# llGuy/madrona_renderer

Measured on AMD Instinct MI355X. Metric: rendered views/sec (whole node), N worlds x 64x64 RGB+depth, higher is better.
Workload: dtype f32

## Files before the change

madrona_renderer_amd/csrc/raster.hip:

```cpp
#include <hip/hip_runtime.h>
#include <algorithm>
#include <cstdlib>

#include "raster.hpp"
#include "raster_dev.hpp"

namespace mrx {
namespace {

constexpr int kWavesPerBlock = 4;
constexpr int kChunk = 64;
constexpr int kHot = 16;
constexpr int kBandRows = 16;
constexpr int kBlocksPerBand = 16;

struct WaveLds {
    float hot[kChunk][kHot];
    float cold[kChunk][kCold];
};

struct TileCtx {
    uint32_t view, tileX0, tileY0;
    uint32_t triBegin, numTris;
    int lx, ly;
};

__device__ __forceinline__ bool tileSetup(const RasterParams &p, uint32_t item, int lane,
                                          TileCtx &t, ViewConst &vc)
{
    const uint32_t tilesPerView = p.tilesFast * p.tilesSlow;
    if (item >= p.numViews * tilesPerView)
        return false;
    t.view = item / tilesPerView;
    const uint32_t tile = item % tilesPerView;
    t.tileX0 = (tile % p.tilesFast) * 64u;
    t.tileY0 = (tile / p.tilesFast) * 64u;
    const float4 q = *reinterpret_cast<const float4 *>(p.camRot + 4 * t.view);
    quatToMat(q.x, q.y, q.z, q.w, vc.Rc);
#pragma unroll
    for (int r = 0; r < 3; ++r) {
        vc.c[r] = p.camPos[3 * t.view + r];
        vc.lv[r] = dot3(vc.Rc[0][r], vc.Rc[1][r], vc.Rc[2][r],
                        p.toLight[0], p.toLight[1], p.toLight[2]);
    }
#pragma unroll
    for (int r = 0; r < 3; ++r) {
#pragma unroll
        for (int cc = 0; cc < 3; ++cc)
            vc.Rc[r][cc] = __uint_as_float(
                __builtin_amdgcn_readfirstlane(__float_as_uint(vc.Rc[r][cc])));
        vc.c[r] = __uint_as_float(__builtin_amdgcn_readfirstlane(__float_as_uint(vc.c[r])));
        vc.lv[r] = __uint_as_float(__builtin_amdgcn_readfirstlane(__float_as_uint(vc.lv[r])));
    }
    t.triBegin = t.view * p.viewTriStride;
    t.numTris = p.viewTriCount[t.view];
    t.lx = lane & 7;
    t.ly = lane >> 3;
    return true;
}

__device__ __forceinline__ uint64_t setupChunk(const RasterParams &p, const ViewConst &vc,
                                               const TileCtx &t, uint32_t chunk, int lane,
                                               WaveLds &L)
{
    bool valid = false;
    const uint32_t k = chunk + lane;
    if (k < t.numTris) {
        const WorldTri wt = p.viewTris[t.triBegin + k];
        TriPlanes c;
        float *h = L.hot[lane];
        valid = setupTriangle(p, vc, wt, (int32_t)k, c, h + 12, L.cold[lane]);
        h[0] = c.A0; h[1] = c.B0; h[2] = c.C0;
        h[3] = c.A1; h[4] = c.B1; h[5] = c.C1;
        h[6] = c.A2; h[7] = c.B2; h[8] = c.C2;
        h[9] = c.Dx; h[10] = c.Dy; h[11] = c.Dc;
    }
    const uint64_t mask = __ballot(valid);
    waveLdsSync();
    return mask;
}

__device__ __forceinline__ const float *shadeRec(const WaveLds &L, int32_t w) { return &L.hot[w][12]; }

template <bool IDS, typename LDS>
__device__ __forceinline__ void resolvePixel(const RasterParams &p, const LDS &L,
                                             int32_t w, float bestInv, float px, float py,
                                             uint32_t &rgba, int32_t &id)
{
    const float *h = shadeRec(L, w);
    rgba = __float_as_uint(h[0]);
    const int32_t tex = __float_as_int(h[1]);
    if (tex >= 0) {
        const float tt = 1.0f / bestInv;
        rgba = shadeTextured(p, L.cold[w], tex, px, py, tt);
    }
    if (IDS)
        id = __float_as_int(p.idsAreSegmask ? h[2] : h[3]);
}

__device__ __forceinline__ void rasterBandBrute(const WaveLds &L, uint64_t validMask,
                                                const float (&pxf)[8], float py0, float py1,
                                                float invNear,
                                                float (&best)[kBlocksPerBand],
                                                int32_t (&bid)[kBlocksPerBand])
{
    for (uint64_t m = validMask; m != 0; m &= m - 1) {
        const int k = __builtin_ctzll(m);
        const float *h = L.hot[k];
        const float A0 = h[0], B0 = h[1], C0 = h[2];
        const float A1 = h[3], B1 = h[4], C1 = h[5];
        const float A2 = h[6], B2 = h[7], C2 = h[8];
        const float Dx = h[9], Dy = h[10], Dc = h[11];
        float r0[2], r1[2], r2[2], rd[2];
        r0[0] = __builtin_fmaf(B0, py0, C0); r0[1] = __builtin_fmaf(B0, py1, C0);
        r1[0] = __builtin_fmaf(B1, py0, C1); r1[1] = __builtin_fmaf(B1, py1, C1);
        r2[0] = __builtin_fmaf(B2, py0, C2); r2[1] = __builtin_fmaf(B2, py1, C2);
        rd[0] = __builtin_fmaf(Dy, py0, Dc); rd[1] = __builtin_fmaf(Dy, py1, Dc);
#pragma unroll
        for (int b = 0; b < kBlocksPerBand; ++b) {
            const int r = b >> 3, bx = b & 7;
            const float e0 = __builtin_fmaf(A0, pxf[bx], r0[r]);
            const float e1 = __builtin_fmaf(A1, pxf[bx], r1[r]);
            const float e2 = __builtin_fmaf(A2, pxf[bx], r2[r]);
            const float it = __builtin_fmaf(Dx, pxf[bx], rd[r]);
            const bool in = (fminf(fminf(e0, e1), e2) >= 0.0f) &&
                            (it > best[b]) && (it <= invNear);
            best[b] = in ? it : best[b];
            bid[b] = in ? k : bid[b];
        }
    }
}

template <bool IDS, bool MULTI, int OUT = kOutRGBD>
__global__ __launch_bounds__(kWave *kWavesPerBlock)
void rasterBruteKernel(const RasterParams p)
{
    __shared__ WaveLds lds[kWavesPerBlock];
    touchKernelArguments();
    const int wave = threadIdx.x / kWave;
    const int lane = threadIdx.x % kWave;
    TileCtx t;
    ViewConst vc;
    if (!tileSetup(p, blockIdx.x * kWavesPerBlock + wave, lane, t, vc))
        return;
    WaveLds &L = lds[wave];

    float pxf[8];
#pragma unroll
    for (int bx = 0; bx < 8; ++bx)
        pxf[bx] = (float)(t.tileX0 + bx * 8 + t.lx);
    const float invNear = p.invNear;

    uint64_t mask0 = 0;
    if (!MULTI)
        mask0 = setupChunk(p, vc, t, 0, lane, L);

    for (int band = 0; band < 4; ++band) {
        float best[kBlocksPerBand];
        int32_t bid[kBlocksPerBand];
        uint32_t outRgba[kBlocksPerBand];
        int32_t outId[kBlocksPerBand];
#pragma unroll
        for (int b = 0; b < kBlocksPerBand; ++b) {
            best[b] = p.invFar;
            bid[b] = -1;
            outRgba[b] = 0xFF000000u;
            outId[b] = -1;
        }
        const float py0 = (float)(t.tileY0 + band * kBandRows + t.ly);
        const float py1 = (float)(t.tileY0 + band * kBandRows + 8 + t.ly);

        if (!MULTI) {
            rasterBandBrute(L, mask0, pxf, py0, py1, invNear, best, bid);
#pragma unroll
            for (int b = 0; b < kBlocksPerBand; ++b)
                if (bid[b] >= 0)
                    resolvePixel<IDS>(p, L, bid[b], best[b], pxf[b & 7],
                                      (b >> 3) ? py1 : py0, outRgba[b], outId[b]);
        } else {
            for (uint32_t chunk = 0; chunk < t.numTris; chunk += kChunk) {
                const uint64_t mask = setupChunk(p, vc, t, chunk, lane, L);
                rasterBandBrute(L, mask, pxf, py0, py1, invNear, best, bid);
#pragma unroll
                for (int b = 0; b < kBlocksPerBand; ++b) {
                    if (bid[b] >= 0)
                        resolvePixel<IDS>(p, L, bid[b], best[b], pxf[b & 7],
                                          (b >> 3) ? py1 : py0, outRgba[b], outId[b]);
                    bid[b] = -1;
                }
                waveLdsSync();
            }
        }

#pragma unroll
        for (int b = 0; b < kBlocksPerBand; ++b) {
            const int r = b >> 3, bx = b & 7;
            const uint32_t fx = t.tileX0 + bx * 8 + t.lx;
            const uint32_t fy = t.tileY0 + band * kBandRows + r * 8 + t.ly;
            if (fx < p.nfast && fy < p.nslow) {
                const bool hit = best[b] > p.invFar;
                const float dep = hit ? 1.0f / best[b] : 0.0f;
                const size_t o = ((size_t)t.view * p.nslow + fy) * p.nfast + fx;
                if (OUT != kOutDepth)
                    p.rgb[o] = outRgba[b];
                if (OUT != kOutRGB)
                    p.depth[o] = dep;
                if (IDS)
                    p.ids[o] = outId[b];
            }
        }
    }
}

constexpr uint32_t kNearFree = 1u << 16;

template <int S0, int S1>
__device__ __forceinline__ uint32_t classifyStrips(const TriPlanes &c, uint32_t tileX0,
                                                   uint32_t tileY0, float invNear, float invFar,
                                                   bool &nearOk)
{
    const float X0 = (float)tileX0, Y0 = (float)tileY0;
    const float xa0 = c.A0 < 0.0f ? X0 : X0 + 31.0f;
    const float xa1 = c.A1 < 0.0f ? X0 : X0 + 31.0f;
    const float xa2 = c.A2 < 0.0f ? X0 : X0 + 31.0f;
    const float xdh = c.Dx < 0.0f ? X0 : X0 + 31.0f;
    const float xdl = c.Dx < 0.0f ? X0 + 31.0f : X0;
    const float yb0 = c.B0 < 0.0f ? Y0 : Y0 + 7.0f;
    const float yb1 = c.B1 < 0.0f ? Y0 : Y0 + 7.0f;
    const float yb2 = c.B2 < 0.0f ? Y0 : Y0 + 7.0f;
    const float ydh = c.Dy < 0.0f ? Y0 : Y0 + 7.0f;
    const float ydl = c.Dy < 0.0f ? Y0 + 7.0f : Y0;
    uint32_t mask = 0;
    float dmax = -__builtin_inff();
#pragma unroll
    for (int s = S0; s < S1; ++s) {
        const float dy = (float)(8 * s);
        const float r0 = __builtin_fmaf(c.B0, yb0 + dy, c.C0);
        const float r1 = __builtin_fmaf(c.B1, yb1 + dy, c.C1);
        const float r2 = __builtin_fmaf(c.B2, yb2 + dy, c.C2);
        const float rh = __builtin_fmaf(c.Dy, ydh + dy, c.Dc);
        const float rl = __builtin_fmaf(c.Dy, ydl + dy, c.Dc);
        const bool yin = (Y0 + dy + 7.0f >= c.bbY0) && (Y0 + dy <= c.bbY1);
#pragma unroll
        for (int hf = 0; hf < 2; ++hf) {
            const float dx = (float)(32 * hf);
            const float e0 = __builtin_fmaf(c.A0, xa0 + dx, r0);
            const float e1 = __builtin_fmaf(c.A1, xa1 + dx, r1);
            const float e2 = __builtin_fmaf(c.A2, xa2 + dx, r2);
            const float dh = __builtin_fmaf(c.Dx, xdh + dx, rh);
            const float dl = __builtin_fmaf(c.Dx, xdl + dx, rl);
            const bool xin = (X0 + dx + 31.0f >= c.bbX0) && (X0 + dx <= c.bbX1);
            const bool possible = (fminf(fminf(e0, e1), e2) >= 0.0f) &&
                                  (dh > invFar) && (dl <= invNear) && xin && yin;
            mask |= possible ? (1u << (2 * s + hf)) : 0u;
            dmax = fmaxf(dmax, dh);
        }
    }
    nearOk = dmax <= invNear;
    return mask;
}

__device__ __forceinline__ uint32_t classifyRegions(const TriPlanes &c, const TileCtx &t,
                                                    float invNear, float invFar)
{
    bool nearOk;
    uint32_t mask = classifyStrips<0, 8>(c, t.tileX0, t.tileY0, invNear, invFar, nearOk);
    if (nearOk)
        mask |= kNearFree;
    return mask;
}


template <bool NEAR>
__device__ __forceinline__ void pixelTest(const PlanePairs &q, f32x2 r01, f32x2 r2d, float px,
                                          float invNear, int32_t kv, float &best, int32_t &bid)
{
    const f32x2 pp = { px, px };
    const f32x2 e01 = fma2(q.A01, pp, r01);
    const f32x2 e2d = fma2(q.A2D, pp, r2d);
    bool in = (fminf(fminf(e01.x, e01.y), e2d.x) >= 0.0f) & (e2d.y > best);
    if (NEAR)
        in = in & (e2d.y <= invNear);
    best = in ? e2d.y : best;
    bid = in ? kv : bid;
}

template <bool NEAR, int IDSHIFT>
__device__ __forceinline__ void rasterRegion(const float (*planes)[16], uint64_t act, int recBase,
                                             const float (&px)[kRegionBlocks], float py,
                                             float invNear,
                                             float (&best)[kRegionBlocks],
                                             int32_t (&bid)[kRegionBlocks])
{
    const f32x2 yy = { py, py };
    for (; act != 0; act &= act - 1) {
        const int k = recBase + __builtin_ctzll(act);
        const PlanePairs q = loadPlanes(planes, k);
        const f32x2 r01 = fma2(q.B01, yy, q.C01);
        const f32x2 r2d = fma2(q.B2D, yy, q.C2D);
#pragma unroll
        for (int b = 0; b < kRegionBlocks; ++b)
            pixelTest<NEAR>(q, r01, r2d, px[b], invNear, k << IDSHIFT, best[b], bid[b]);
    }
}

template <bool IDS>
__device__ __forceinline__ void outputRegion(const RasterParams &p, const TileCtx &t,
                                             uint32_t fx0, uint32_t fy, float invFar,
                                             const float (&best)[kRegionBlocks],
                                             const uint32_t (&rgba)[kRegionBlocks],
                                             const int32_t (&id)[kRegionBlocks])
{
    float dep[kRegionBlocks];
#pragma unroll
    for (int b = 0; b < kRegionBlocks; ++b)
        dep[b] = best[b] > invFar ? __builtin_amdgcn_rcpf(best[b]) : 0.0f;
    if (fy >= p.nslow || (p.debugSkip & 1u))
        return;
    const size_t o = ((size_t)t.view * p.nslow + fy) * p.nfast + fx0;
    const bool doRgb = storesRgb<kOutByPointer>(p.rgb), doDepth = storesDepth<kOutByPointer>(p.depth);
    if ((p.nfast & 3u) == 0 && fx0 + 3 < p.nfast) {
        if (doRgb)
            streamStore16(p.writeThrough, p.rgb + o, rgba[0], rgba[1], rgba[2], rgba[3]);
        if (doDepth)
            streamStore16(p.writeThrough, p.depth + o, __float_as_uint(dep[0]), __float_as_uint(dep[1]),
                          __float_as_uint(dep[2]), __float_as_uint(dep[3]));
        if (IDS)
            streamStore16(p.writeThrough, p.ids + o, (uint32_t)id[0], (uint32_t)id[1], (uint32_t)id[2], (uint32_t)id[3]);
    } else {
#pragma unroll
        for (int b = 0; b < kRegionBlocks; ++b) {
            if (fx0 + b < p.nfast) {
                if (doRgb)
                    streamStore4(p.writeThrough, p.rgb + o + b, rgba[b]);
                if (doDepth)
                    streamStore4(p.writeThrough, p.depth + o + b, __float_as_uint(dep[b]));
                if (IDS)
                    streamStore4(p.writeThrough, p.ids + o + b, (uint32_t)id[b]);
            }
        }
    }
}

constexpr int kPass = kChunk * kWavesPerBlock;

struct PassRecs {
    float shade[kPass][4];
    float cold[kPass][kCold];
};
struct TileLds {
    float planes[kPass][16];
    PassRecs rec;
};
__device__ __forceinline__ const float *shadeRec(const PassRecs &L, int32_t w) { return L.shade[w]; }

template <bool IDS>
__global__ __launch_bounds__(kWave *kWavesPerBlock, 3)
void rasterChunkedKernel(const RasterParams p)
{
    __shared__ TileLds lds;
    touchKernelArguments();
    const int wave = threadIdx.x / kWave;
    const int lane = threadIdx.x % kWave;
    TileCtx t;
    ViewConst vc;
    if (!tileSetup(p, blockIdx.x, lane, t, vc))
        return;
    const float invNear = p.invNear, invFar = p.invFar;

    float best[4][kRegionBlocks];
    int32_t bid[4][kRegionBlocks];
    uint32_t outRgba[4][kRegionBlocks];
    int32_t outId[4][kRegionBlocks];
#pragma unroll
    for (int g = 0; g < 4; ++g)
#pragma unroll
        for (int b = 0; b < kRegionBlocks; ++b) {
            best[g][b] = invFar;
            bid[g][b] = -1;
            outRgba[g][b] = 0xFF000000u;
            outId[g][b] = -1;
        }

    for (uint32_t pass = 0; pass < t.numTris; pass += kPass) {
        if (pass != 0)
            __syncthreads();
        {
            const int rec = wave * kWave + lane;
            const uint32_t k = pass + (uint32_t)rec;
            TriPlanes c;
            c.A0 = c.B0 = c.C0 = c.A1 = c.B1 = c.C1 = 0.0f;
            c.A2 = c.B2 = c.C2 = c.Dx = c.Dy = c.Dc = 0.0f;
            c.bbX0 = c.bbX1 = c.bbY0 = c.bbY1 = 0.0f;
            uint32_t mask = 0;
            if (pass + (uint32_t)(wave * kWave) < t.numTris) {
                bool valid = false;
                if (k < t.numTris && !(p.debugSkip & 8u)) {
                    const WorldTri wt = p.viewTris[t.triBegin + k];
                    valid = setupTriangle(p, vc, wt, (int32_t)k, c, lds.rec.shade[rec], lds.rec.cold[rec]);
                }
                if (valid && !(p.debugSkip & 4u))
                    mask = classifyRegions(c, t, invNear, invFar);
            }
            float4 *dst = reinterpret_cast<float4 *>(lds.planes[rec]);
            dst[0] = make_float4(c.A0, c.A1, c.A2, c.Dx);
            dst[1] = make_float4(c.B0, c.B1, c.B2, c.Dy);
            dst[2] = make_float4(c.C0, c.C1, c.C2, c.Dc);
            dst[3] = make_float4(__uint_as_float(mask), 0.f, 0.f, 0.f);
        }
        __syncthreads();

        const uint32_t left = t.numTris - pass;
        const int subs = left >= (uint32_t)kPass ? kWavesPerBlock : (int)((left + kWave - 1) / kWave);
#pragma unroll
        for (int g = 0; g < 4; ++g) {
            const int strip = 2 * wave + (g >> 1), hf = g & 1;
            const uint32_t fy = t.tileY0 + strip * 8 + t.ly;
            const float py = (float)fy;
            const uint32_t fx0 = t.tileX0 + hf * 32 + 4 * t.lx;
            float px[kRegionBlocks];
#pragma unroll
            for (int b = 0; b < kRegionBlocks; ++b)
                px[b] = (float)(fx0 + b);
            for (int sub = 0; sub < subs; ++sub) {
                const uint32_t mask = __float_as_uint(lds.planes[sub * kWave + lane][12]);
                const uint64_t act = __ballot((mask >> (2 * strip + hf)) & 1u);
                if (!(p.debugSkip & 2u))
                    rasterRegion<true, 0>(lds.planes, act, sub * kWave, px, py, invNear, best[g], bid[g]);
            }
#pragma unroll
            for (int b = 0; b < kRegionBlocks; ++b) {
                if (bid[g][b] >= 0)
                    resolvePixel<IDS>(p, lds.rec, bid[g][b], best[g][b], px[b], py,
                                      outRgba[g][b], outId[g][b]);
                bid[g][b] = -1;
            }
        }
    }

#pragma unroll
    for (int g = 0; g < 4; ++g) {
        const int strip = 2 * wave + (g >> 1), hf = g & 1;
        const uint32_t fy = t.tileY0 + strip * 8 + t.ly;
        const uint32_t fx0 = t.tileX0 + hf * 32 + 4 * t.lx;
        outputRegion<IDS>(p, t, fx0, fy, invFar, best[g], outRgba[g], outId[g]);
    }
}

constexpr int kGroupTilesMax = 16;
constexpr int kGroupSlotsMax = 256;
constexpr int groupTilesMax(int slots) { return slots <= 128 ? kGroupTilesMax : 8; }

template <int SLOTS>
struct GroupLds {
    static constexpr int kRecs = SLOTS <= kChunk ? kChunk + 16 : SLOTS;
    static constexpr int kBackground = kRecs;
    float planes[kRecs][16];
    uint32_t live[kRecs];
    float shade[kRecs + 1][4];
    float cold[kRecs][kCold];
    uint32_t masks[groupTilesMax(SLOTS) * (SLOTS <= kChunk ? kChunk : SLOTS)];
    uint32_t tileInfo[kGroupTilesMax][4];
    uint32_t nextItem;
    uint8_t itemOrder[kGroupTilesMax * 8];
};
constexpr uint32_t kTileValid = 4u;


template <bool IDS, bool FULL, bool TEX, int OUT, typename LDS>
__device__ __forceinline__ void storeRegion(const RasterParams &p, const LDS &L, bool doRgb, bool doDepth,
                                            uint32_t *rgbTile, float *depthTile, int32_t *idsTile,
                                            uint32_t pixOff, uint32_t fx0, uint32_t fy,
                                            bool anyTex, const float (&px)[kRegionBlocks], float py,
                                            const float (&best)[kRegionBlocks],
                                            const int32_t (&bid)[kRegionBlocks])
{
    uint32_t rgba[kRegionBlocks];
    int32_t id[kRegionBlocks];
    float dep[kRegionBlocks];
    const char *shadeBase = reinterpret_cast<const char *>(&L.shade[0][0]);
#pragma unroll
    for (int b = 0; b < kRegionBlocks; ++b) {
        const float *h = reinterpret_cast<const float *>(shadeBase + bid[b]);
        if (OUT != kOutDepth)
            rgba[b] = __float_as_uint(h[0]);
        if (IDS)
            id[b] = __float_as_int(p.idsAreSegmask ? h[2] : h[3]);
        if (OUT != kOutRGB)
            dep[b] = bid[b] != LDS::kBackground * 16 ? __builtin_amdgcn_rcpf(best[b]) : 0.0f;
    }
    if (TEX && OUT != kOutDepth && anyTex && (OUT != kOutByPointer || doRgb)) {
#pragma unroll
        for (int b = 0; b < kRegionBlocks; ++b) {
            const int32_t rec = bid[b] >> 4;
            const int32_t tex = __float_as_int(L.shade[rec][1]);
            if (tex >= 0)
                rgba[b] = shadeTextured(p, L.cold[rec], tex, px[b], py, 1.0f / best[b]);
        }
    }
    if (p.debugSkip & 1u)
        return;
    if (FULL) {
        if (doRgb)
            streamStore16(p.writeThrough, rgbTile + pixOff, rgba[0], rgba[1], rgba[2], rgba[3]);
        if (doDepth)
            streamStore16(p.writeThrough, depthTile + pixOff, __float_as_uint(dep[0]), __float_as_uint(dep[1]),
                          __float_as_uint(dep[2]), __float_as_uint(dep[3]));
        if (IDS)
            streamStore16(p.writeThrough, idsTile + pixOff, (uint32_t)id[0], (uint32_t)id[1], (uint32_t)id[2], (uint32_t)id[3]);
    } else if (fy < p.nslow) {
#pragma unroll
        for (int b = 0; b < kRegionBlocks; ++b) {
            if (fx0 + b < p.nfast) {
                if (doRgb)
                    streamStore4(p.writeThrough, rgbTile + pixOff + b, rgba[b]);
                if (doDepth)
                    streamStore4(p.writeThrough, depthTile + pixOff + b, __float_as_uint(dep[b]));
                if (IDS)
                    streamStore4(p.writeThrough, idsTile + pixOff + b, (uint32_t)id[b]);
            }
        }
    }
}

template <bool IDS, bool FULL>
__device__ __forceinline__ void storeBackground(const RasterParams &p, bool doRgb, bool doDepth, uint32_t *rgbTile,
                                                float *depthTile, int32_t *idsTile,
                                                uint32_t pixOff, uint32_t fx0, uint32_t fy)
{
    if (p.debugSkip & 1u)
        return;
    const uint32_t bg = 0xFF000000u;
    if (FULL) {
        if (doRgb)
            streamStore16(p.writeThrough, rgbTile + pixOff, bg, bg, bg, bg);
        if (doDepth)
            streamStore16(p.writeThrough, depthTile + pixOff, 0u, 0u, 0u, 0u);
        if (IDS)
            streamStore16(p.writeThrough, idsTile + pixOff, ~0u, ~0u, ~0u, ~0u);
    } else if (fy < p.nslow) {
#pragma unroll
        for (int b = 0; b < kRegionBlocks; ++b) {
            if (fx0 + b < p.nfast) {
                if (doRgb)
                    streamStore4(p.writeThrough, rgbTile + pixOff + b, bg);
                if (doDepth)
                    streamStore4(p.writeThrough, depthTile + pixOff + b, 0u);
                if (IDS)
                    streamStore4(p.writeThrough, idsTile + pixOff + b, ~0u);
            }
        }
    }
}

struct GroupSetupArgs {
    const ObjTri *tris;
    const TriMat *triMats;
    const float *instPos, *instRot, *instScale;
    float sx, ox, sz, oz, s6bPad, ambient, diffuse;
    int32_t transposed;
};

constexpr int groupWaves(bool tex) { return tex ? 4 : 8; }

template <bool IDS, int SLOTS, bool TEX, int XMODE, bool FAST, int OUT>
__device__ __forceinline__ void groupKernelBody(const char *hPose, const char *hGeom, uint32_t hViews, uint32_t hInstances,
                                                uint32_t hPool, uint32_t hShape, uint32_t hGroups, uint32_t hPrefix,
                                                uint32_t hFirst01, uint32_t hFirst23, const RasterParams p)
{
    __shared__ GroupLds<SLOTS> lds;
    constexpr int kBackground = GroupLds<SLOTS>::kBackground;
    const int wave = __builtin_amdgcn_readfirstlane(threadIdx.x / kWave);
    const int lane = threadIdx.x % kWave;
    if (!FAST || wave >= 2)
        touchKernelArguments<(FAST ? 48 : 0) + sizeof(RasterParams)>();
    const uint32_t aNumViews = FAST ? hViews : p.numViews;
    const uint32_t aGrpViews = FAST ? (hShape & 255u) : p.grpViews;
    const uint32_t aXcdSkew = FAST ? ((hShape >> 8) & 15u) : p.xcdSkew;
    const uint32_t aXcdRotate = FAST ? ((hShape >> 12) & 1u) : p.xcdRotate;
    const uint32_t aGrpPerView = FAST ? 1u : p.grpPerView;
    const uint32_t aGrid = FAST ? hGroups : gridDim.x;
    const uint32_t aUniInstances = FAST ? ((hShape >> 13) & 7u) : p.uniInstances;
    const uint32_t aUniCams = FAST ? ((hShape >> 16) & 255u) : p.uniCamsPerWorld;
    const uint32_t dskip = FAST ? 0u : p.debugSkip;
    const PoseLayout lay = poseLayout(hViews, hInstances);
    const float *aCamRot = FAST ? reinterpret_cast<const float *>(hPose + lay.camRot) : p.camRot;
    const float *aCamPos = FAST ? reinterpret_cast<const float *>(hPose + lay.camPos) : p.camPos;
    const int32_t *aInstObj = FAST ? reinterpret_cast<const int32_t *>(hPose + lay.instObj) : p.instObj;
    const uint32_t tilesPerView = FAST ? 1u : p.tilesFast * p.tilesSlow;
    uint32_t firstView, groupViews, firstTile, groupTiles;
    const uint32_t blk = ((XMODE & 1) && SLOTS == 16 && aXcdSkew && (blockIdx.x ^ 1u) < aGrid)
                             ? blockIdx.x ^ 1u : blockIdx.x;
    if ((XMODE & 2) && blockIdx.x == 0 && threadIdx.x == (groupWaves(TEX) - 1) * kWave && p.xccReport)
        *p.xccReport = __builtin_amdgcn_s_getreg((3 << 11) | 20);
    uint32_t bid = blk;
    if (aXcdRotate && (bid | 7u) < aGrid)
        bid = (bid & ~7u) | ((bid + 2u * (bid >> 3)) & 7u);
    if (aGrpPerView == 1) {
        firstView = bid * aGrpViews;
        groupViews = aGrpViews;
        firstTile = 0;
        groupTiles = groupViews * tilesPerView;
    } else {
        firstView = bid / aGrpPerView;
        groupViews = 1;
        firstTile = (bid - firstView * aGrpPerView) * p.grpChunkTiles;
        groupTiles = min(p.grpChunkTiles, tilesPerView - firstTile);
    }
    uint32_t firstStrip = 0, numStrips = groupTiles * 8;
    if (SLOTS == 16 && aXcdSkew) {
        if (blk & 1u) {
            firstStrip = aXcdSkew;
            numStrips -= aXcdSkew;
        } else {
            groupViews += 1;
            groupTiles += 1;
            numStrips += aXcdSkew;
        }
    }
    const int groupRecs = (int)groupViews * SLOTS;
    const int numPairs = (int)groupTiles * SLOTS;
    const float invNear = p.invNear, invFar = p.invFar;
    if (dskip & 16u)
        return;
    unsigned long long *stamps = (!FAST && p.debugStamps && wave < 4)
        ? p.debugStamps + ((size_t)blockIdx.x * 4 + wave) * 8 : nullptr;
#define MRX_STAMP(i)                                                           \
    do {                                                                       \
        if (stamps && lane == 0)                                               \
            stamps[i] = __builtin_amdgcn_s_memrealtime();                      \
    } while (0)
    MRX_STAMP(0);
    for (int i = threadIdx.x; i < numPairs; i += groupWaves(TEX) * kWave)
        lds.masks[i] = 0u;

    if (wave == groupWaves(TEX) - 1 && lane < (int)groupTiles) {
        uint32_t vi = (uint32_t)lane, tile = firstTile;
        if (tilesPerView != 1) {
            vi = groupViews == 1 ? 0u : (uint32_t)lane / tilesPerView;
            tile = firstTile + (uint32_t)lane - vi * tilesPerView;
        }
        const uint32_t ty = tilesPerView != 1 ? tile / p.tilesFast : 0u;
        lds.tileInfo[lane][0] = firstView + vi;
        lds.tileInfo[lane][1] = (tile - ty * p.tilesFast) * 64u;
        lds.tileInfo[lane][2] = ty * 64u;
        lds.tileInfo[lane][3] = (firstView + vi < aNumViews ? kTileValid : 0u) | ((vi * SLOTS) << 8);
    }
    if (wave == groupWaves(TEX) - 1) {
        uint32_t base = 0;
        for (uint32_t c0 = 0; c0 < groupTiles * 8u; c0 += kWave) {
            const uint32_t c = c0 + (uint32_t)lane;
            uint32_t strip = c / groupTiles, tile = c - strip * groupTiles;
            if (tilesPerView != 1) {
                tile = c >> 3;
                strip = c & 7u;
            }
            const uint32_t g = tile * 8u + strip;
            const bool ok = strip < 8u && g >= firstStrip && g < firstStrip + numStrips;
            const uint64_t m = __ballot(ok);
            if (ok)
                lds.itemOrder[base + __builtin_popcountll(m & ((1ull << lane) - 1ull))] = (uint8_t)g;
            base += (uint32_t)__builtin_popcountll(m);
        }
    }
    if (wave * kWave < groupRecs) {
        const int rec = wave * kWave + lane;
        const int vi = rec / SLOTS, k = rec % SLOTS;
        const bool recOk = rec < groupRecs;
        const bool viewOk = recOk && firstView + vi < aNumViews;
        const uint32_t view = viewOk ? firstView + vi : 0u;
        WorldTri wt;
        uint32_t numTris;
        if (aUniInstances) {
            const uint32_t kk = (uint32_t)k;
            const uint32_t pre1 = FAST ? (hPrefix & 255u) : p.uniPrefix[1], pre2 = FAST ? ((hPrefix >> 8) & 255u) : p.uniPrefix[2];
            const uint32_t pre3 = FAST ? ((hPrefix >> 16) & 255u) : p.uniPrefix[3], pre4 = FAST ? (hPrefix >> 24) : p.uniPrefix[4];
            const uint32_t ft0 = FAST ? (hFirst01 & 0xFFFFu) : p.uniFirstTri[0], ft1 = FAST ? (hFirst01 >> 16) : p.uniFirstTri[1];
            const uint32_t ft2 = FAST ? (hFirst23 & 0xFFFFu) : p.uniFirstTri[2], ft3 = FAST ? (hFirst23 >> 16) : p.uniFirstTri[3];
            const uint32_t li = (kk >= pre1 ? 1u : 0u) + (kk >= pre2 ? 1u : 0u) + (kk >= pre3 ? 1u : 0u);
            const uint32_t pre = li == 0 ? 0u : li == 1 ? pre1 : li == 2 ? pre2 : pre3;
            const uint32_t first = li == 0 ? ft0 : li == 1 ? ft1 : li == 2 ? ft2 : ft3;
            uint32_t world = view;
            if (aUniCams != 1)
                world = view / aUniCams;
            wt.inst = world * aUniInstances + li;
            wt.tri = first + (kk - pre);
            numTris = viewOk ? pre4 : 0u;
            if (kk >= pre4) {
                wt.inst = 0;
                wt.tri = 0;
            }
        } else {
            wt = p.viewTris[view * p.viewTriStride + ((uint32_t)k < p.viewTriStride ? (uint32_t)k : 0u)];
            numTris = viewOk ? p.viewTriCount[view] : 0u;
        }
        ViewConst vc;
        {
            const float4 q = *reinterpret_cast<const float4 *>(aCamRot + 4 * view);
            quatToMat(q.x, q.y, q.z, q.w, vc.Rc);
#pragma unroll
            for (int r = 0; r < 3; ++r) {
                vc.c[r] = aCamPos[3 * view + r];
                vc.lv[r] = dot3(vc.Rc[0][r], vc.Rc[1][r], vc.Rc[2][r],
                                p.toLight[0], p.toLight[1], p.toLight[2]);
            }
        }
        TriPlanes c;
        c.A0 = c.B0 = c.C0 = c.A1 = c.B1 = c.C1 = 0.0f;
        c.A2 = c.B2 = c.C2 = c.Dx = c.Dy = c.Dc = 0.0f;
        c.bbX0 = c.bbX1 = c.bbY0 = c.bbY1 = 0.0f;
        bool valid = false;
        MRX_STAMP(1);
        if (recOk) {
            lds.shade[rec][1] = __int_as_float(-1);
            if ((uint32_t)k < numTris && !(dskip & 8u)) {
                const GroupSetupArgs sa = {
                    FAST ? reinterpret_cast<const ObjTri *>(hGeom) : p.tris,
                    FAST ? reinterpret_cast<const TriMat *>(hGeom + geomMatsOffset(hPool)) : p.triMats,
                    FAST ? reinterpret_cast<const float *>(hPose + lay.instPos) : p.instPos,
                    FAST ? reinterpret_cast<const float *>(hPose + lay.instRot) : p.instRot,
                    FAST ? reinterpret_cast<const float *>(hPose + lay.instScale) : p.instScale,
                    p.sx, p.ox, p.sz, p.oz, p.s6bPad, p.ambient, p.diffuse, p.transposed };
                InstXform x;
                instanceTransform(sa, vc, wt.inst, x);
                valid = setupTriangleCore<true, OUT != kOutDepth>(sa, vc.lv, x, wt.tri, aInstObj[wt.inst], k, c,
                                                                  lds.shade[rec], lds.cold[rec]);
            }
            MRX_STAMP(2);
            float4 *dst = reinterpret_cast<float4 *>(lds.planes[rec]);
            dst[0] = make_float4(c.A0, c.A1, c.A2, c.Dx);
            dst[1] = make_float4(c.B0, c.B1, c.B2, c.Dy);
            dst[2] = make_float4(c.C0, c.C1, c.C2, c.Dc);
            dst[3] = make_float4(c.bbX0, c.bbX1, c.bbY0, c.bbY1);
            lds.live[rec] = (valid && !(dskip & 4u)) ? 1u : 0u;
        }
        if (rec == 0) {
            lds.nextItem = 0;
            lds.shade[kBackground][0] = __uint_as_float(0xFF000000u);
            lds.shade[kBackground][1] = __int_as_float(-1);
            lds.shade[kBackground][2] = __int_as_float(-1);
            lds.shade[kBackground][3] = __int_as_float(-1);
        }
    }
    __syncthreads();
    MRX_STAMP(3);

    constexpr int kPairStride = (groupWaves(TEX) / 4) * kWave;
    for (int pair = (wave >> 2) * kWave + lane; pair - lane < numPairs; pair += kPairStride) {
        if (pair >= numPairs)
            continue;
        const int j = pair / SLOTS, k = pair % SLOTS;
        const uint32_t info = lds.tileInfo[j][3];
        const int rec = (int)(info >> 8) + k;
        if (!(info & kTileValid) || !lds.live[rec])
            continue;
        const float4 *src = reinterpret_cast<const float4 *>(lds.planes[rec]);
        const float4 a = src[0], b = src[1], cc = src[2], bb = src[3];
        TriPlanes c;
        c.A0 = a.x; c.A1 = a.y; c.A2 = a.z; c.Dx = a.w;
        c.B0 = b.x; c.B1 = b.y; c.B2 = b.z; c.Dy = b.w;
        c.C0 = cc.x; c.C1 = cc.y; c.C2 = cc.z; c.Dc = cc.w;
        c.bbX0 = bb.x; c.bbX1 = bb.y; c.bbY0 = bb.z; c.bbY1 = bb.w;
        const uint32_t tx0 = lds.tileInfo[j][1], ty0 = lds.tileInfo[j][2];
        bool nearOk = false;
        uint32_t m;
        switch (wave & 3) {
        case 0: m = classifyStrips<0, 2>(c, tx0, ty0, invNear, invFar, nearOk); break;
        case 1: m = classifyStrips<2, 4>(c, tx0, ty0, invNear, invFar, nearOk); break;
        case 2: m = classifyStrips<4, 6>(c, tx0, ty0, invNear, invFar, nearOk); break;
        default: m = classifyStrips<6, 8>(c, tx0, ty0, invNear, invFar, nearOk); break;
        }
        if (nearOk)
            m |= 1u << (16 + (wave & 3));
        if (m)
            atomicOr(&lds.masks[pair], m);
    }
    __syncthreads();
    MRX_STAMP(4);

    const int lx = lane & 7, ly = lane >> 3;
    const uint32_t laneOff = (uint32_t)ly * p.nfast + 4u * lx;
    int cachedTile = -1, recBase = 0;
    constexpr int SUBS = (SLOTS + kWave - 1) / kWave;
    constexpr int LANES = SLOTS < kWave ? SLOTS : kWave;
    uint32_t view = 0, tileX0 = 0, tileY0 = 0, mask[SUBS] = {};
    float pxTile[2][kRegionBlocks] = {};
    bool anyTex = false, nearFree = false, full = false;
    uint32_t *rgbTile = nullptr;
    float *depthTile = nullptr;
    int32_t *idsTile = nullptr;
    const bool doRgb = storesRgb<OUT>(p.rgb), doDepth = storesDepth<OUT>(p.depth);
    for (;;) {
        uint32_t item = 0;
        if (lane == 0)
            item = atomicAdd(&lds.nextItem, 1u);
        item = __builtin_amdgcn_readfirstlane(item);
        if (item >= numStrips)
            break;
        item = __builtin_amdgcn_readfirstlane((uint32_t)lds.itemOrder[item]);
        const int j = (int)(item >> 3), strip = (int)(item & 7u);
        if (j != cachedTile) {
            const uint32_t info = __builtin_amdgcn_readfirstlane(lds.tileInfo[j][3]);
            if (!(info & kTileValid))
                continue;
            cachedTile = j;
            recBase = (int)(info >> 8);
            view = __builtin_amdgcn_readfirstlane(lds.tileInfo[j][0]);
            tileX0 = __builtin_amdgcn_readfirstlane(lds.tileInfo[j][1]);
            tileY0 = __builtin_amdgcn_readfirstlane(lds.tileInfo[j][2]);
            const size_t tileBase = ((size_t)view * p.nslow + tileY0) * p.nfast + tileX0;
            rgbTile = p.rgb + tileBase;
            depthTile = p.depth + tileBase;
            idsTile = IDS ? p.ids + tileBase : nullptr;
            full = (p.nfast & 3u) == 0 && tileX0 + 64u <= p.nfast && tileY0 + 64u <= p.nslow;
            anyTex = false;
            nearFree = true;
#pragma unroll
            for (int sub = 0; sub < SUBS; ++sub) {
                const int slot = sub * kWave + lane;
                mask[sub] = lane < LANES ? lds.masks[j * SLOTS + slot] : 0u;
                const int32_t tex = lane < LANES ? __float_as_int(lds.shade[recBase + slot][1]) : -1;
                anyTex = anyTex || __ballot((mask[sub] & 0xFFFFu) != 0 && tex >= 0) != 0;
                nearFree = nearFree &&
                           __ballot((mask[sub] & 0xFFFFu) != 0 && ((mask[sub] >> 16) & 0xFu) != 0xFu) == 0;
            }
#pragma unroll
            for (int hf = 0; hf < 2; ++hf)
#pragma unroll
                for (int b = 0; b < kRegionBlocks; ++b)
                    pxTile[hf][b] = (float)(tileX0 + hf * 32 + 4 * lx + b);
        }
        const uint32_t fy = tileY0 + strip * 8 + ly;
        const float py = (float)fy;
#pragma unroll
        for (int hf = 0; hf < 2; ++hf) {
            const uint32_t fx0 = tileX0 + hf * 32 + 4 * lx;
            const uint32_t pixOff = (uint32_t)(strip * 8) * p.nfast + hf * 32 + laneOff;
            uint64_t act[SUBS];
            bool any = false;
#pragma unroll
            for (int sub = 0; sub < SUBS; ++sub) {
                act[sub] = __ballot((mask[sub] >> (2 * strip + hf)) & 1u);
                any = any || act[sub] != 0;
            }
            if (!any) {
                if (full)
                    storeBackground<IDS, true>(p, doRgb, doDepth, rgbTile, depthTile, idsTile, pixOff, fx0, fy);
                else
                    storeBackground<IDS, false>(p, doRgb, doDepth, rgbTile, depthTile, idsTile, pixOff, fx0, fy);
                continue;
            }
            const float (&px)[kRegionBlocks] = pxTile[hf];
            float best[kRegionBlocks];
            int32_t bid[kRegionBlocks];
#pragma unroll
            for (int b = 0; b < kRegionBlocks; ++b) {
                best[b] = invFar;
                bid[b] = kBackground * 16;
            }
            if (!(dskip & 2u)) {
#pragma unroll
                for (int sub = 0; sub < SUBS; ++sub) {
                    if (SUBS > 1 && act[sub] == 0)
                        continue;
                    if (nearFree)
                        rasterRegion<false, 4>(lds.planes, act[sub], recBase + sub * kWave, px, py, invNear, best, bid);
                    else
                        rasterRegion<true, 4>(lds.planes, act[sub], recBase + sub * kWave, px, py, invNear, best, bid);
                }
            }
            if (full)
                storeRegion<IDS, true, TEX, OUT>(p, lds, doRgb, doDepth, rgbTile, depthTile, idsTile, pixOff, fx0, fy,
                                            anyTex, px, py, best, bid);
            else
                storeRegion<IDS, false, TEX, OUT>(p, lds, doRgb, doDepth, rgbTile, depthTile, idsTile, pixOff, fx0, fy,
                                             anyTex, px, py, best, bid);
        }
    }
    MRX_STAMP(5);
    MRX_STAMP(6);
    if (stamps && lane == 0)
        stamps[7] = ((unsigned long long)__builtin_amdgcn_s_getreg((31 << 11) | 20) << 32) |
                    (unsigned long long)__builtin_amdgcn_s_getreg((31 << 11) | 4);
#undef MRX_STAMP
}

template <bool IDS, int SLOTS, bool TEX, int XMODE = 0, int OUT = kOutRGBD>
__global__ __launch_bounds__(kWave *groupWaves(TEX), TEX ? (SLOTS > 128 ? 3 : 4) : (SLOTS > 128 ? 6 : 8))
void rasterGroupKernel(const RasterParams p)
{
    groupKernelBody<IDS, SLOTS, TEX, XMODE, false, OUT>(nullptr, nullptr, 0u, 0u, 0u, 0u, 0u, 0u, 0u, 0u, p);
}

template <bool IDS, bool TEX, int XMODE, int OUT>
__global__ __launch_bounds__(kWave *groupWaves(TEX), TEX ? 4 : 8)
void rasterGroupKernelFast(const char *hPose, const char *hGeom, uint32_t hViews, uint32_t hInstances, uint32_t hPool,
                           uint32_t hShape, uint32_t hGroups, uint32_t hPrefix, uint32_t hFirst01, uint32_t hFirst23,
                           const RasterParams p)
{
    groupKernelBody<IDS, 16, TEX, XMODE, true, OUT>(hPose, hGeom, hViews, hInstances, hPool, hShape, hGroups, hPrefix, hFirst01,
                                               hFirst23, p);
}

}

hipError_t launchRaster(const RasterParams &p, uint32_t maxWorldTris,
                        int32_t variant, hipStream_t stream)
{
    const uint32_t items = p.numViews * p.tilesFast * p.tilesSlow;
    if (items == 0)
        return hipSuccess;
    const dim3 block(kWave * kWavesPerBlock);
    const bool ids = p.ids != nullptr;
    const bool multi = maxWorldTris > (uint32_t)kChunk;
    const bool large = maxWorldTris > (uint32_t)kGroupSlotsMax;
    if (variant == kVariantBrute) {
        const dim3 grid((items + kWavesPerBlock - 1) / kWavesPerBlock);
#define MRX_BRUTE(O)                                                                     \
    do {                                                                                 \
        if (ids) {                                                                       \
            if (multi) rasterBruteKernel<true, true, O><<<grid, block, 0, stream>>>(p);   \
            else       rasterBruteKernel<true, false, O><<<grid, block, 0, stream>>>(p);  \
        } else {                                                                         \
            if (multi) rasterBruteKernel<false, true, O><<<grid, block, 0, stream>>>(p);  \
            else       rasterBruteKernel<false, false, O><<<grid, block, 0, stream>>>(p); \
        }                                                                                \
    } while (0)
        const OutSel out = outSelOf(p.rgb, p.depth);
        if (out == kOutDepth)    MRX_BRUTE(kOutDepth);
        else if (out == kOutRGB) MRX_BRUTE(kOutRGB);
        else                     MRX_BRUTE(kOutRGBD);
#undef MRX_BRUTE
    } else if (large) {
        if (ids) rasterChunkedKernel<true><<<dim3(items), block, 0, stream>>>(p);
        else     rasterChunkedKernel<false><<<dim3(items), block, 0, stream>>>(p);
    } else {
        int slots = 16;
        while ((uint32_t)slots < maxWorldTris)
            slots *= 2;
        if (p.debugSlots >= slots && p.debugSlots <= kGroupSlotsMax && (p.debugSlots & (p.debugSlots - 1)) == 0)
            slots = p.debugSlots;
        const uint32_t tpv = p.tilesFast * p.tilesSlow;
        const uint32_t maxTiles = (uint32_t)groupTilesMax(slots);
        const uint32_t kFill = groupFill(p.numCUs);
        RasterParams q = p;
        uint32_t vg = 1, ct = tpv, gpv = 1;
        if (tpv == 1) {
            vg = std::max<uint32_t>(1u, (uint32_t)(kChunk / slots));
            if (p.anyTextured)
                vg = std::min<uint32_t>(vg, 2u);
            while (vg > 1 && (p.numViews + vg - 1) / vg < (vg == 2 ? kFill / 2 : kFill))
                vg /= 2;
        } else if (p.anyTextured) {
            ct = std::max<uint32_t>(1u, std::min<uint32_t>(4u, tpv / 4u));
        } else {
            ct = std::min<uint32_t>(tpv, std::min<uint32_t>(maxTiles, 8u));
        }
        if (tpv != 1)
            while (ct > 1 && (uint64_t)p.numViews * ((tpv + ct - 1) / ct) < kFill)
                ct = (ct + 1) / 2;
        if (p.grpViewsWanted > 0 && tpv * (uint32_t)p.grpViewsWanted <= maxTiles &&
            p.grpViewsWanted * slots <= kChunk) {
            vg = (uint32_t)p.grpViewsWanted;
            ct = tpv;
        }
        if (p.grpTilesWanted > 0 && (uint32_t)p.grpTilesWanted <= maxTiles) {
            vg = 1;
            ct = std::min<uint32_t>((uint32_t)p.grpTilesWanted, tpv);
        }
        gpv = (tpv + ct - 1) / ct;
        q.grpViews = vg;
        q.grpChunkTiles = ct;
        q.grpPerView = gpv;
        const uint32_t numGroups = gpv == 1 ? (p.numViews + vg - 1) / vg : p.numViews * gpv;
        const bool skewable = slots == 16 && tpv == 1 && (vg == 4 || vg == 2);
        q.xcdSkew = (skewable && numGroups >= kFill) ? (vg == 4 ? 3u : 1u) : 0u;
        if (p.xcdSkewWanted >= 0)
            q.xcdSkew = skewable ? (uint32_t)(p.xcdSkewWanted < 8 ? p.xcdSkewWanted : 7) : 0u;
        q.xcdRotate = (tpv == 1 && numGroups >= kFill) ? 1u : 0u;
        if (p.xcdRotateWanted >= 0)
            q.xcdRotate = p.xcdRotateWanted ? 1u : 0u;
        const dim3 grid(numGroups);
        const dim3 gblock(kWave * groupWaves(p.anyTextured != 0));
        GroupHeader h {};
        h.pose = p.poseBlock;
        h.geom = p.geomBlock;
        h.views = p.numViews;
        h.instances = p.numInstances;
        h.poolTris = p.poolTris;
        h.groups = numGroups;
        bool fast = slots == 16 && tpv == 1 && gpv == 1 && p.uniInstances != 0 && p.uniCamsPerWorld < 256 && vg < 256 &&
                    p.poseBlock && p.geomBlock && p.debugSkip == 0 && p.debugStamps == nullptr && p.uniPrefix[4] < 256;
        for (int i = 0; i < 4 && fast; ++i)
            fast = p.uniFirstTri[i] < 65536u;
        if (const char *dbg = std::getenv("MRX_GROUP_FAST"))
            fast = fast && std::atoi(dbg) != 0;
        if (fast) {
            h.shape = vg | (q.xcdSkew << 8) | (q.xcdRotate << 12) | (p.uniInstances << 13) | (p.uniCamsPerWorld << 16) | (1u << 31);
            h.prefix = p.uniPrefix[1] | (p.uniPrefix[2] << 8) | (p.uniPrefix[3] << 16) | (p.uniPrefix[4] << 24);
            h.first01 = p.uniFirstTri[0] | (p.uniFirstTri[1] << 16);
            h.first23 = p.uniFirstTri[2] | (p.uniFirstTri[3] << 16);
        }
#define MRX_GROUP_ARGS h.pose, h.geom, h.views, h.instances, h.poolTris, h.shape, h.groups, h.prefix, h.first01, h.first23, q
#define MRX_GROUP_O(S, X, O, OP)                                               \
    do {                                                                       \
        if (fast && S == 16) {                                                 \
            if (p.anyTextured) {                                               \
                if (ids) rasterGroupKernelFast<true, true, X, O><<<grid, gblock, 0, stream>>>(MRX_GROUP_ARGS);   \
                else     rasterGroupKernelFast<false, true, X, O><<<grid, gblock, 0, stream>>>(MRX_GROUP_ARGS);  \
            } else {                                                           \
                if (ids) rasterGroupKernelFast<true, false, X, O><<<grid, gblock, 0, stream>>>(MRX_GROUP_ARGS);  \
                else     rasterGroupKernelFast<false, false, X, O><<<grid, gblock, 0, stream>>>(MRX_GROUP_ARGS); \
            }                                                                  \
        } else if (p.anyTextured) {                                            \
            if (ids) rasterGroupKernel<true, S, true, X, OP><<<grid, gblock, 0, stream>>>(q);   \
            else     rasterGroupKernel<false, S, true, X, OP><<<grid, gblock, 0, stream>>>(q);  \
        } else {                                                               \
            if (ids) rasterGroupKernel<true, S, false, X, OP><<<grid, gblock, 0, stream>>>(q);  \
            else     rasterGroupKernel<false, S, false, X, OP><<<grid, gblock, 0, stream>>>(q); \
        }                                                                      \
    } while (0)
        const OutSel out = outSelOf(p.rgb, p.depth);
#define MRX_GROUP_X(S, X)                                                      \
    do {                                                                       \
        if (out == kOutDepth)    MRX_GROUP_O(S, X, kOutDepth, kOutDepth);      \
        else if (out == kOutRGB) MRX_GROUP_O(S, X, kOutRGB, kOutByPointer);    \
        else                     MRX_GROUP_O(S, X, kOutRGBD, kOutRGBD);        \
    } while (0)
#define MRX_GROUP(S) MRX_GROUP_X(S, 0)
        if (slots == 16) {
            const int xmode = ((q.xcdSkew && (p.xcdPhase & 1u)) ? 1 : 0) | (p.xccReport ? 2 : 0);
            if (xmode == 0) MRX_GROUP_X(16, 0);
            else if (xmode == 1) MRX_GROUP_X(16, 1);
            else if (xmode == 2) MRX_GROUP_X(16, 2);
            else MRX_GROUP_X(16, 3);
        }
        else if (slots == 32) MRX_GROUP(32);
        else if (slots == 64) MRX_GROUP(64);
        else if (slots == 128) MRX_GROUP(128);
        else MRX_GROUP(256);
#undef MRX_GROUP_ARGS
#undef MRX_GROUP_X
#undef MRX_GROUP_O
#undef MRX_GROUP
    }
    return hipGetLastError();
}

}
```

Before: 178.9 million.

## Precompute per-strip work items with ballot masks during classification for fast path

For the FAST non-textured path, the classify phase now ballots per-strip left/right coverage masks and the near-free and any-texture flags, then writes a ready-made item descriptor per strip into LDS at a precomputed position. The raster loop reads one uint2 per item instead of reloading per-tile masks and recomputing flags with ballots on every tile change, and the mask-clearing pass is skipped. This removes per-item LDS reads and ballot work in the hot loop. In exchange it adds ballots and LDS writes to classification and relies on 64x64 single-tile views and 16 slots (j fits in 4 bits, tile origin at 0).

```diff
diff --git a/madrona_renderer_amd/csrc/raster.hip b/madrona_renderer_amd/csrc/raster.hip
--- a/madrona_renderer_amd/csrc/raster.hip
+++ b/madrona_renderer_amd/csrc/raster.hip
@@ -463,8 +463,13 @@
     uint32_t tileInfo[kGroupTilesMax][4];
     uint32_t nextItem;
     uint8_t itemOrder[kGroupTilesMax * 8];
+    uint2 items[SLOTS == 16 ? kGroupTilesMax * 8 : 1];
+    uint8_t itemPos[SLOTS == 16 ? kGroupTilesMax * 8 : 1];
 };
 constexpr uint32_t kTileValid = 4u;
+constexpr uint32_t kItemValid = 1u << 8;
+constexpr uint32_t kItemNearFree = 1u << 9;
+constexpr uint32_t kItemAnyTex = 1u << 10;
 
 
 template <bool IDS, bool FULL, bool TEX, int OUT, typename LDS>
@@ -551,6 +556,35 @@
             }
         }
     }
+}
+
+template <typename LDS>
+__device__ __forceinline__ uint32_t classifyPair(const LDS &L, int j, int k, int wave, float invNear, float invFar,
+                                                 bool &nearOk, bool &tex)
+{
+    nearOk = false;
+    tex = false;
+    const uint32_t info = L.tileInfo[j][3];
+    const int rec = (int)(info >> 8) + k;
+    if (!(info & kTileValid) || !L.live[rec])
+        return 0u;
+    const float4 *src = reinterpret_cast<const float4 *>(L.planes[rec]);
+    const float4 a = src[0], b = src[1], cc = src[2], bb = src[3];
+    TriPlanes c;
+    c.A0 = a.x; c.A1 = a.y; c.A2 = a.z; c.Dx = a.w;
+    c.B0 = b.x; c.B1 = b.y; c.B2 = b.z; c.Dy = b.w;
+    c.C0 = cc.x; c.C1 = cc.y; c.C2 = cc.z; c.Dc = cc.w;
+    c.bbX0 = bb.x; c.bbX1 = bb.y; c.bbY0 = bb.z; c.bbY1 = bb.w;
+    const uint32_t tx0 = L.tileInfo[j][1], ty0 = L.tileInfo[j][2];
+    uint32_t m;
+    switch (wave & 3) {
+    case 0: m = classifyStrips<0, 2>(c, tx0, ty0, invNear, invFar, nearOk); break;
+    case 1: m = classifyStrips<2, 4>(c, tx0, ty0, invNear, invFar, nearOk); break;
+    case 2: m = classifyStrips<4, 6>(c, tx0, ty0, invNear, invFar, nearOk); break;
+    default: m = classifyStrips<6, 8>(c, tx0, ty0, invNear, invFar, nearOk); break;
+    }
+    tex = __float_as_int(L.shade[rec][1]) >= 0;
+    return m;
 }
 
 struct GroupSetupArgs {
@@ -588,6 +622,7 @@
     const float *aCamPos = FAST ? reinterpret_cast<const float *>(hPose + lay.camPos) : p.camPos;
     const int32_t *aInstObj = FAST ? reinterpret_cast<const int32_t *>(hPose + lay.instObj) : p.instObj;
     const uint32_t tilesPerView = FAST ? 1u : p.tilesFast * p.tilesSlow;
+    constexpr bool readyItems = FAST && !TEX;
     uint32_t firstView, groupViews, firstTile, groupTiles;
     const uint32_t blk = ((XMODE & 1) && SLOTS == 16 && aXcdSkew && (blockIdx.x ^ 1u) < aGrid)
                              ? blockIdx.x ^ 1u : blockIdx.x;
@@ -631,8 +666,9 @@
             stamps[i] = __builtin_amdgcn_s_memrealtime();                      \
     } while (0)
     MRX_STAMP(0);
-    for (int i = threadIdx.x; i < numPairs; i += groupWaves(TEX) * kWave)
-        lds.masks[i] = 0u;
+    if (!readyItems)
+        for (int i = threadIdx.x; i < numPairs; i += groupWaves(TEX) * kWave)
+            lds.masks[i] = 0u;
 
     if (wave == groupWaves(TEX) - 1 && lane < (int)groupTiles) {
         uint32_t vi = (uint32_t)lane, tile = firstTile;
@@ -658,8 +694,13 @@
             const uint32_t g = tile * 8u + strip;
             const bool ok = strip < 8u && g >= firstStrip && g < firstStrip + numStrips;
             const uint64_t m = __ballot(ok);
-            if (ok)
-                lds.itemOrder[base + __builtin_popcountll(m & ((1ull << lane) - 1ull))] = (uint8_t)g;
+            const uint32_t pos = base + __builtin_popcountll(m & ((1ull << lane) - 1ull));
+            if (readyItems) {
+                if (strip < 8u)
+                    lds.itemPos[g] = ok ? (uint8_t)pos : (uint8_t)0xFF;
+            } else if (ok) {
+                lds.itemOrder[pos] = (uint8_t)g;
+            }
             base += (uint32_t)__builtin_popcountll(m);
         }
     }
@@ -747,29 +788,37 @@
 
     constexpr int kPairStride = (groupWaves(TEX) / 4) * kWave;
     for (int pair = (wave >> 2) * kWave + lane; pair - lane < numPairs; pair += kPairStride) {
+        if (readyItems) {
+            uint32_t m = 0;
+            bool nearOk = false, tex = false;
+            if (pair < numPairs)
+                m = classifyPair(lds, pair / SLOTS, pair % SLOTS, wave, invNear, invFar, nearOk, tex);
+            m >>= 4 * (wave & 3);
+            const uint64_t l0 = __ballot(m & 1u), r0 = __ballot(m & 2u), l1 = __ballot(m & 4u), r1 = __ballot(m & 8u);
+            const uint64_t near0 = __ballot((m & 3u) && !nearOk), near1 = __ballot((m & 12u) && !nearOk);
+            const uint64_t tex0 = __ballot((m & 3u) && tex), tex1 = __ballot((m & 12u) && tex);
+            if (lane % 16 == 0 && pair < numPairs) {
+                const uint32_t j = (uint32_t)pair / 16u;
+                const uint32_t valid = firstView + j < aNumViews ? kItemValid : 0u;
+                const auto put = [&](uint32_t strip, uint64_t l, uint64_t r, uint64_t nearHit, uint64_t texHit) {
+                    const uint32_t pos = lds.itemPos[j * 8u + strip];
+                    if (pos == 0xFFu)
+                        return;
+                    const uint32_t desc = j | strip << 4 | valid |
+                                          (((nearHit >> lane) & 0xFFFFu) == 0 ? kItemNearFree : 0u) |
+                                          (((texHit >> lane) & 0xFFFFu) != 0 ? kItemAnyTex : 0u);
+                    lds.items[pos] = make_uint2((uint32_t)((l >> lane) & 0xFFFFu) | (uint32_t)((r >> lane) & 0xFFFFu) << 16,
+                                                desc);
+                };
+                put(2u * (wave & 3), l0, r0, near0, tex0);
+                put(2u * (wave & 3) + 1u, l1, r1, near1, tex1);
+            }
+            continue;
+        }
         if (pair >= numPairs)
             continue;
-        const int j = pair / SLOTS, k = pair % SLOTS;
-        const uint32_t info = lds.tileInfo[j][3];
-        const int rec = (int)(info >> 8) + k;
-        if (!(info & kTileValid) || !lds.live[rec])
-            continue;
-        const float4 *src = reinterpret_cast<const float4 *>(lds.planes[rec]);
-        const float4 a = src[0], b = src[1], cc = src[2], bb = src[3];
-        TriPlanes c;
-        c.A0 = a.x; c.A1 = a.y; c.A2 = a.z; c.Dx = a.w;
-        c.B0 = b.x; c.B1 = b.y; c.B2 = b.z; c.Dy = b.w;
-        c.C0 = cc.x; c.C1 = cc.y; c.C2 = cc.z; c.Dc = cc.w;
-        c.bbX0 = bb.x; c.bbX1 = bb.y; c.bbY0 = bb.z; c.bbY1 = bb.w;
-        const uint32_t tx0 = lds.tileInfo[j][1], ty0 = lds.tileInfo[j][2];
-        bool nearOk = false;
-        uint32_t m;
-        switch (wave & 3) {
-        case 0: m = classifyStrips<0, 2>(c, tx0, ty0, invNear, invFar, nearOk); break;
-        case 1: m = classifyStrips<2, 4>(c, tx0, ty0, invNear, invFar, nearOk); break;
-        case 2: m = classifyStrips<4, 6>(c, tx0, ty0, invNear, invFar, nearOk); break;
-        default: m = classifyStrips<6, 8>(c, tx0, ty0, invNear, invFar, nearOk); break;
-        }
+        bool nearOk, tex;
+        uint32_t m = classifyPair(lds, pair / SLOTS, pair % SLOTS, wave, invNear, invFar, nearOk, tex);
         if (nearOk)
             m |= 1u << (16 + (wave & 3));
         if (m)
@@ -790,6 +839,15 @@
     float *depthTile = nullptr;
     int32_t *idsTile = nullptr;
     const bool doRgb = storesRgb<OUT>(p.rgb), doDepth = storesDepth<OUT>(p.depth);
+    uint32_t itemMasks = 0;
+    if (readyItems) {
+        full = (p.nfast & 3u) == 0 && 64u <= p.nfast && 64u <= p.nslow;
+#pragma unroll
+        for (int hf = 0; hf < 2; ++hf)
+#pragma unroll
+            for (int b = 0; b < kRegionBlocks; ++b)
+                pxTile[hf][b] = (float)(hf * 32 + 4 * lx + b);
+    }
     for (;;) {
         uint32_t item = 0;
         if (lane == 0)
@@ -797,38 +855,57 @@
         item = __builtin_amdgcn_readfirstlane(item);
         if (item >= numStrips)
             break;
-        item = __builtin_amdgcn_readfirstlane((uint32_t)lds.itemOrder[item]);
-        const int j = (int)(item >> 3), strip = (int)(item & 7u);
-        if (j != cachedTile) {
-            const uint32_t info = __builtin_amdgcn_readfirstlane(lds.tileInfo[j][3]);
-            if (!(info & kTileValid))
+        int j, strip;
+        if (readyItems) {
+            const uint2 d = lds.items[item];
+            itemMasks = __builtin_amdgcn_readfirstlane(d.x);
+            const uint32_t desc = __builtin_amdgcn_readfirstlane(d.y);
+            if (!(desc & kItemValid))
                 continue;
-            cachedTile = j;
-            recBase = (int)(info >> 8);
-            view = __builtin_amdgcn_readfirstlane(lds.tileInfo[j][0]);
-            tileX0 = __builtin_amdgcn_readfirstlane(lds.tileInfo[j][1]);
-            tileY0 = __builtin_amdgcn_readfirstlane(lds.tileInfo[j][2]);
-            const size_t tileBase = ((size_t)view * p.nslow + tileY0) * p.nfast + tileX0;
+            j = (int)(desc & 15u);
+            strip = (int)((desc >> 4) & 7u);
+            nearFree = (desc & kItemNearFree) != 0;
+            anyTex = (desc & kItemAnyTex) != 0;
+            recBase = j * SLOTS;
+            const size_t tileBase = (size_t)(firstView + (uint32_t)j) * p.nslow * p.nfast;
             rgbTile = p.rgb + tileBase;
             depthTile = p.depth + tileBase;
             idsTile = IDS ? p.ids + tileBase : nullptr;
-            full = (p.nfast & 3u) == 0 && tileX0 + 64u <= p.nfast && tileY0 + 64u <= p.nslow;
-            anyTex = false;
-            nearFree = true;
-#pragma unroll
-            for (int sub = 0; sub < SUBS; ++sub) {
-                const int slot = sub * kWave + lane;
-                mask[sub] = lane < LANES ? lds.masks[j * SLOTS + slot] : 0u;
-                const int32_t tex = lane < LANES ? __float_as_int(lds.shade[recBase + slot][1]) : -1;
-                anyTex = anyTex || __ballot((mask[sub] & 0xFFFFu) != 0 && tex >= 0) != 0;
-                nearFree = nearFree &&
-                           __ballot((mask[sub] & 0xFFFFu) != 0 && ((mask[sub] >> 16) & 0xFu) != 0xFu) == 0;
-            }
-#pragma unroll
-            for (int hf = 0; hf < 2; ++hf)
-#pragma unroll
-                for (int b = 0; b < kRegionBlocks; ++b)
-                    pxTile[hf][b] = (float)(tileX0 + hf * 32 + 4 * lx + b);
+        } else {
+            item = __builtin_amdgcn_readfirstlane((uint32_t)lds.itemOrder[item]);
+            j = (int)(item >> 3);
+            strip = (int)(item & 7u);
+            if (j != cachedTile) {
+                const uint32_t info = __builtin_amdgcn_readfirstlane(lds.tileInfo[j][3]);
+                if (!(info & kTileValid))
+                    continue;
+                cachedTile = j;
+                recBase = (int)(info >> 8);
+                view = __builtin_amdgcn_readfirstlane(lds.tileInfo[j][0]);
+                tileX0 = __builtin_amdgcn_readfirstlane(lds.tileInfo[j][1]);
+                tileY0 = __builtin_amdgcn_readfirstlane(lds.tileInfo[j][2]);
+                const size_t tileBase = ((size_t)view * p.nslow + tileY0) * p.nfast + tileX0;
+                rgbTile = p.rgb + tileBase;
+                depthTile = p.depth + tileBase;
+                idsTile = IDS ? p.ids + tileBase : nullptr;
+                full = (p.nfast & 3u) == 0 && tileX0 + 64u <= p.nfast && tileY0 + 64u <= p.nslow;
+                anyTex = false;
+                nearFree = true;
+#pragma unroll
+                for (int sub = 0; sub < SUBS; ++sub) {
+                    const int slot = sub * kWave + lane;
+                    mask[sub] = lane < LANES ? lds.masks[j * SLOTS + slot] : 0u;
+                    const int32_t tex = lane < LANES ? __float_as_int(lds.shade[recBase + slot][1]) : -1;
+                    anyTex = anyTex || __ballot((mask[sub] & 0xFFFFu) != 0 && tex >= 0) != 0;
+                    nearFree = nearFree &&
+                               __ballot((mask[sub] & 0xFFFFu) != 0 && ((mask[sub] >> 16) & 0xFu) != 0xFu) == 0;
+                }
+#pragma unroll
+                for (int hf = 0; hf < 2; ++hf)
+#pragma unroll
+                    for (int b = 0; b < kRegionBlocks; ++b)
+                        pxTile[hf][b] = (float)(tileX0 + hf * 32 + 4 * lx + b);
+            }
         }
         const uint32_t fy = tileY0 + strip * 8 + ly;
         const float py = (float)fy;
@@ -840,7 +917,8 @@
             bool any = false;
 #pragma unroll
             for (int sub = 0; sub < SUBS; ++sub) {
-                act[sub] = __ballot((mask[sub] >> (2 * strip + hf)) & 1u);
+                act[sub] = readyItems ? (uint64_t)((itemMasks >> (16 * hf)) & 0xFFFFu)
+                                     : __ballot((mask[sub] >> (2 * strip + hf)) & 1u);
                 any = any || act[sub] != 0;
             }
             if (!any) {
```

Result: faster. 186.3 million (median of 6 runs) (+4.2%).
